# in3otd/glfer

Measured on NVIDIA B200. Metric: spectrogram_frames_per_sec, higher is better.
Workload: dtype f32

## Files before the change

glfer_b200/csrc/gram_common.cuh:

```cuda
#pragma once
#include <cuda_runtime.h>
#include <cstdio>
#include <cstdlib>
#include <cstring>
#include <cstdint>
#include <atomic>
#include <vector>
#include <algorithm>

#include "fft_core.cuh"
#include "fft_wpf.cuh"
#include "levels.cuh"
#include "avg_frame.cuh"
#include "tables.hpp"
#include "../../include/glb_shim.h"

using namespace glb;

extern std::atomic<unsigned long long> g_launches;
extern int g_big_pair;
extern int g_kernel_pref;
extern int g_last_family;
extern "C" void glb_set_error(const char *msg);

// ... 762 lines not shown
        last_pass_rt<M>(v, t, buf, p.tw, tr);
        if (MULTI) {
          if (w0) emit_bins_rt<M, true>(v, t, tr, sink_multi);
          else emit_bins_rt<M, false>(v, t, tr, sink_multi);
        } else {
          if (w0) emit_bins_rt<M, true>(v, t, tr, sink_single);
          else emit_bins_rt<M, false>(v, t, tr, sink_single);
        }
      } else {
        TwRegs tl;
        load_last_regs<M>(tl, t, p.tw, p.vtab);
        last_pass_load<M>(v, t, buf);
        last_pass_compute_rt<M>(v, t, tl);
        if (MULTI) {
          if (w0) emit_bins_rt<M, true>(v, t, tl, sink_multi);
          else emit_bins_rt<M, false>(v, t, tl, sink_multi);
        } else {
          if (w0) emit_bins_rt<M, true>(v, t, tl, sink_single);
          else emit_bins_rt<M, false>(v, t, tl, sink_single);
        }
      }
      if (!MULTI) {
        if constexpr (LEV) {
          if (active) store_levels<M>(lev_ptr, t, yv, p.lm);
        }
        if (!LEV || p.rows != nullptr) {
          if (db) {
#pragma unroll
            for (int slot = 0; slot < 17; slot++) yv[slot] = 10.f * log10f(yv[slot]);
          }
          if constexpr (AVG) {
            if (active && av_mask != 0) {
              float *hrow = hist + hslot * av_band - p.av.minbin;
#pragma unroll
              for (int slot = 0; slot < 17; slot++)
                if (av_mask & (1u << slot)) hrow[slot_bin<M>(t, slot)] = yv[slot];
            }
          }
          if (active && storing) {
            GLB_CHECK_ROW(p, row);
            GLB_CHECK_ROW(p, row + M);
            store_row<M>(row, t, yv);
          }
        }
      }
    }
    if (MULTI && active) {
      float *row = row_ptr;
      const bool db = p.rows_db != 0;
      if constexpr (LEV) store_levels<M>(lev_ptr, t, acc, p.lm);
      if (!LEV || p.rows != nullptr) {
#pragma unroll
        for (int slot = 0; slot < 17; slot++) {
          if (slot < 16 || t == 0) {
            float y = acc[slot];
            if (db) y = 10.f * log10f(y);
            row[slot_bin<M>(t, slot)] = y;
          }
        }
      }
    }
    slot_new = slot_next;
    if constexpr (AVG) hslot = (hslot + 1 == av_depth) ? 0 : hslot + 1;
  }
}



template <int M, int P> struct PairMidPasses {
  static __device__ __forceinline__ void run(float2 (&va)[kPoints], float2 (&vb)[kPoints], int t, float4 *buf, const TwRegs &tr) {
    if constexpr (P < Plan<M>::NP - 1) {
      pass_load2<M>(va, vb, t, buf);
      pass_compute_rt<M, P>(va, tr);
      pass_compute_rt<M, P>(vb, tr);
      __syncthreads();
      pass_scatter2<M, P>(va, vb, t, buf);
      __syncthreads();
      PairMidPasses<M, P + 1>::run(va, vb, t, buf, tr);
    }
  }
};

template <int M, int QS> struct PairGeo {
  static constexpr int T = M / kPoints, NB = kPoints >> QS, SLOTS = NB + 1, NW = (T + 31) / 32;
  static constexpr int HOP = (2 * T) << QS;
  static constexpr int G = Geo<M>::G, THREADS = Geo<M>::THREADS;
  static constexpr size_t BUF_BYTES = (size_t) BufSize<M>::value * sizeof(float4);
  static constexpr size_t RING_OFF = BUF_BYTES;
  static constexpr size_t RED_OFF = RING_OFF + (size_t) SLOTS * HOP * sizeof(float);
  static constexpr size_t MU_OFF = RED_OFF + (((size_t) (NB + 1) * NW * sizeof(float) + 15) / 16) * 16;
  static constexpr size_t MBAR_OFF = MU_OFF + (((size_t) SLOTS * sizeof(float) + 15) / 16) * 16;
  static constexpr size_t GROUP_BYTES = MBAR_OFF + 16;
  static constexpr size_t SMEM = (size_t) G * GROUP_BYTES;
  static constexpr int MINB_ = 65536 / (THREADS * 168);
  static constexpr int MINB = MINB_ < 1 ? 1 : MINB_;
};

template <int M, int QS>
__global__ void __launch_bounds__(Geo<M>::THREADS, (PairGeo<M, QS>::MINB)) gram_pair_kernel(const KParams p) {
  using PG = PairGeo<M, QS>;
  constexpr int T = PG::T, G = PG::G, N = 2 * M, NB = PG::NB, SLOTS = PG::SLOTS, NW = PG::NW, HOP = PG::HOP;
  constexpr int BQ = 1 << QS;
  constexpr int W = T < 32 ? T : 32;
  extern __shared__ __align__(16) unsigned char smem_raw[];
  const int g = threadIdx.x / T;
  const int t = threadIdx.x % T;
  unsigned char *gbase = smem_raw + (size_t) g * PG::GROUP_BYTES;
  float4 *buf = reinterpret_cast<float4 *>(gbase);
  float *ring = reinterpret_cast<float *>(gbase + PG::RING_OFF);
  float *red = reinterpret_cast<float *>(gbase + PG::RED_OFF);
  float *mu = reinterpret_cast<float *>(gbase + PG::MU_OFF);
  unsigned long long *mbar = reinterpret_cast<unsigned long long *>(gbase + PG::MBAR_OFF);
  const long long gid = (long long) blockIdx.x * G + g;
  const long long fb = gid * p.frames_per_group;
  const bool group_active = fb < p.nframes;
  const long long f_first = p.first_frame + fb;
  const bool sub = p.fused_mean != 0;
  constexpr unsigned blk_bytes = (unsigned) HOP * 4u;
  unsigned phase = 0;

  TwRegs tr;
  load_tw_regs<M>(tr, t, p.tw, p.vtab);

  if (t == 0) {
    mbar_init(mbar, 1);
    asm volatile("fence.mbarrier_init.release.cluster;" ::: "memory");
  }
  __syncthreads();

  {
    const long long b0 = f_first - (NB - 1);
    const bool b_there = fb + 1 < p.nframes;
    unsigned bytes = 0;
#pragma unroll
    for (int lb = 0; lb <= NB; lb++) {
      const long long blk = b0 + lb;
      const bool want = group_active && blk >= 0 && (lb < NB || b_there);
      if (!want) {
        float2 *z = reinterpret_cast<float2 *>(ring + (size_t) lb * HOP);
#pragma unroll
        for (int i = 0; i < BQ; i++) z[t + T * i] = make_float2(0.f, 0.f);
      } else {
        bytes += blk_bytes;
      }
    }
    if (bytes != 0) {
      if (t == 0) {
        mbar_expect_tx(mbar, bytes);
#pragma unroll
        for (int lb = 0; lb <= NB; lb++) {
          const long long blk = b0 + lb;
          if (blk >= 0 && (lb < NB || b_there))
            tma_load_1d(ring + (size_t) lb * HOP, p.samples + (blk * HOP - p.origin), blk_bytes, mbar);
        }
      }
      mbar_wait(mbar, phase);
      phase ^= 1;
    }
    __syncthreads();
    if (sub) {
#pragma unroll
      for (int lb = 0; lb < NB - 1; lb++) {
        const float m = ring_block_mean<M>(ring + (size_t) lb * HOP, QS, t, red + lb * NW, p.inv_hop_mean, g);
        if (t == 0) mu[lb] = m;
      }
      __syncthreads();
    }
  }

  int s0 = 0;
  bool pending = false;
  for (int it = 0; it < p.frames_per_group; it += 2) {
    const long long fl = fb + it;
    const bool active_a = fl < p.nframes, active_b = fl + 1 < p.nframes;
    const long long f = p.first_frame + fl;
    if (pending) {
      mbar_wait(mbar, phase);
      phase ^= 1;
    }
    int slot_of[NB + 1];
#pragma unroll
    for (int lb = 0; lb <= NB; lb++) slot_of[lb] = (s0 + lb) % SLOTS;

    float2 va[kPoints], vb[kPoints];
    {
      float2 x[kPoints + BQ];
#pragma unroll
      for (int lb = 0; lb <= NB; lb++) {
        const float2 *bp = reinterpret_cast<const float2 *>(ring + (size_t) slot_of[lb] * HOP);
#pragma unroll
        for (int i = 0; i < BQ; i++) x[lb * BQ + i] = bp[t + T * i];
      }
      float m[NB + 1];
#pragma unroll
      for (int lb = 0; lb <= NB; lb++) m[lb] = 0.f;
      if (sub) {
        float sn[2];
#pragma unroll
        for (int e = 0; e < 2; e++) {
          float a = 0.f;
#pragma unroll
          for (int i = 0; i < BQ; i++) {
            const float2 c = x[(NB - 1 + e) * BQ + i];
            a += c.x + c.y;
          }
#pragma unroll
          for (int o = W / 2; o > 0; o >>= 1) a += __shfl_xor_sync(0xffffffffu, a, o);
          sn[e] = a;
        }
        if (NW > 1) {
          if ((t & 31) == 0) {
            red[t >> 5] = sn[0];
            red[NW + (t >> 5)] = sn[1];
          }
          __syncthreads();
        }
        m[NB - 1] = ring_block_total<M>(sn[0], red, p.inv_hop_mean);
        m[NB] = ring_block_total<M>(sn[1], red + NW, p.inv_hop_mean);
#pragma unroll
        for (int lb = 0; lb < NB - 1; lb++) m[lb] = mu[slot_of[lb]];
        if (t == 0) {
          mu[slot_of[NB - 1]] = m[NB - 1];
          mu[slot_of[NB]] = m[NB];
        }
      }
      const float2 *w2 = reinterpret_cast<const float2 *>(p.tapers);
#pragma unroll
      for (int q = 0; q < kPoints; q++) {
        const float2 w = ld_taper(w2 + t + T * q);
        va[q] = mul2(sub2(x[q], bc(m[q >> QS])), w);
        vb[q] = mul2(sub2(x[q + BQ], bc(m[(q >> QS) + 1])), w);
      }
    }
    pass_compute_rt<M, 0>(va, tr);
    pass_compute_rt<M, 0>(vb, tr);
    __syncthreads();
    pass_scatter2<M, 0>(va, vb, t, buf);
    {
      const bool next_a = (it + 2 < p.frames_per_group) && (fl + 2 < p.nframes);
      const bool next_b = next_a && (fl + 3 < p.nframes);
      pending = next_a;
      if (next_a && t == 0) {
        asm volatile("fence.proxy.async.shared::cta;" ::: "memory");
        mbar_expect_tx(mbar, next_b ? 2 * blk_bytes : blk_bytes);
        tma_load_1d(ring + (size_t) slot_of[0] * HOP, p.samples + ((f + 2) * (long long) HOP - p.origin), blk_bytes, mbar);
        if (next_b)
          tma_load_1d(ring + (size_t) slot_of[1] * HOP, p.samples + ((f + 3) * (long long) HOP - p.origin), blk_bytes, mbar);
      }
    }
    __syncthreads();
    PairMidPasses<M, 1>::run(va, vb, t, buf, tr);
    last_pass_load2<M>(va, vb, t, buf);
    const bool db = p.rows_db != 0;
    const bool w0 = t < 32;
#pragma unroll
    for (int e = 0; e < 2; e++) {
      float2 *v = e == 0 ? va : vb;
      last_pass_compute_rt<M>(v, t, tr);
      float yv[17];
      yv[16] = 1.f;
      auto sink = [&](int slot, float2 a, bool) { yv[slot] = norm2(a); };
      if (w0) emit_bins_rt<M, true>(v, t, tr, sink);
      else emit_bins_rt<M, false>(v, t, tr, sink);
      if (db) {
#pragma unroll
        for (int slot = 0; slot < 17; slot++) yv[slot] = 10.f * log10f(yv[slot]);
      }
      if (e == 0 ? active_a : active_b) store_row<M>(p.rows + (fl + e) * p.row_stride, t, yv);
    }
    s0 = (s0 + 2) % SLOTS;
  }
}

#ifndef GLB_WPF_MINB
#define GLB_WPF_MINB 5
#endif
constexpr int kWpfWarps = 2;

template <int M, int QW>
__device__ __forceinline__ void wpf_remove_means(float2 (&x)[kWP], float inv_hop) {
  constexpr int T = Wpf<M>::T, NB = kWP >> QW;
#pragma unroll
  for (int b = 0; b < NB; b++) {
    float s = 0.f;
#pragma unroll
    for (int q = b << QW; q < (b + 1) << QW; q++) s += x[q].x + x[q].y;
#pragma unroll
    for (int o = T / 2; o > 0; o >>= 1) s += __shfl_xor_sync(0xffffffffu, s, o);
    const float m = s * inv_hop;
#pragma unroll
    for (int q = b << QW; q < (b + 1) << QW; q++) {
      x[q].x -= m;
      x[q].y -= m;
    }
  }
}

template <int M>
__global__ void __launch_bounds__(32 * kWpfWarps, GLB_WPF_MINB) gram_wpf_kernel(const KParams p) {
  constexpr int T = Wpf<M>::T, N = 2 * M, FPW = 32 / T;
  extern __shared__ __align__(16) unsigned char smem_raw[];
  const int warp = threadIdx.x >> 5, lane = threadIdx.x & 31;
  const int g = lane / T, t = lane % T;
  float2 *tile = reinterpret_cast<float2 *>(smem_raw) + (size_t) (warp * FPW + g) * (Wpf<M>::TILE + 2);
  const long long gid = ((long long) blockIdx.x * kWpfWarps + warp) * FPW + g;
  const long long fb = gid * p.frames_per_group;

  WpfRegs rg;
  wpf_load_regs<M>(rg, t, p.roots, p.vtab);
  const float2 *w2 = reinterpret_cast<const float2 *>(p.tapers) + t;
  const bool db = p.rows_db != 0;

  for (int it = 0; it < p.frames_per_group; ++it) {
    const long long fl = fb + it;
    const bool active = fl < p.nframes;
    const long long fe = active ? fl : (p.nframes - 1);
    const long long f = p.first_frame + fe;
    const float2 *src = reinterpret_cast<const float2 *>(p.samples + (f * (long long) p.hop - p.n_ov - p.origin)) + t;
    float2 v[kWP];
#pragma unroll
    for (int q = 0; q < kWP; q++) v[q] = ldg2(src + T * q);
    if (fl + 1 < p.nframes && it + 1 < p.frames_per_group) {
      const float *nx = p.samples + ((f + 1) * (long long) p.hop - p.origin);
      for (int i = t * 32; i < p.hop; i += T * 32) asm volatile("prefetch.global.L2 [%0];" ::"l"(nx + i));
    }
    if (p.fused_mean) {
      switch (p.qs) {
        case 6: wpf_remove_means<M, 6>(v, p.inv_hop_mean); break;
        case 5: wpf_remove_means<M, 5>(v, p.inv_hop_mean); break;
        case 4: wpf_remove_means<M, 4>(v, p.inv_hop_mean); break;
        case 3: wpf_remove_means<M, 3>(v, p.inv_hop_mean); break;
        default: wpf_remove_means<M, 2>(v, p.inv_hop_mean); break;
      }
    }
#pragma unroll
    for (int q = 0; q < kWP; q++) {
      const float2 w = ldg2(w2 + T * q);
      v[q].x *= w.x;
      v[q].y *= w.y;
    }
    wpf_pass_a<M>(v);
    __syncwarp();
    wpf_scatter<M>(v, t, tile);
    __syncwarp();
    wpf_gather<M>(v, t, tile);
    wpf_pass_b<M>(v, t, rg);
    float *row = p.rows + fe * p.row_stride;
    wpf_emit<M>(v, t, rg, [&](int, int bin, float2 a, bool) {
      float y = norm2(a);
      if (db) y = 10.f * log10f(y);
      if (active) row[bin] = y;
    });
  }
}

template <int M>
inline int launch_wpf(const KParams &kp, cudaStream_t st) {
  int dev = 0, sms = 0;
  CU(cudaGetDevice(&dev));
  CU(cudaDeviceGetAttribute(&sms, cudaDevAttrMultiProcessorCount, dev));
  constexpr int FPW = 32 / Wpf<M>::T;
  const size_t smem = (size_t) kWpfWarps * FPW * (Wpf<M>::TILE + 2) * sizeof(float2);
  static thread_local int occ_cache[64];
  int &occ = occ_cache[dev & 63];
  if (occ == 0) {
    CU(cudaFuncSetAttribute(gram_wpf_kernel<M>, cudaFuncAttributeMaxDynamicSharedMemorySize, 227 * 1024));
    CU(cudaOccupancyMaxActiveBlocksPerMultiprocessor(&occ, gram_wpf_kernel<M>, 32 * kWpfWarps, smem));
    if (occ < 1) occ = 1;
  }
  long long groups = (long long) sms * occ * kWpfWarps * FPW;
  if (groups > kp.nframes) groups = kp.nframes;
  if (groups < 1) groups = 1;
  KParams k = kp;
  k.frames_per_group = (int) ((kp.nframes + groups - 1) / groups);
  const long long used = (kp.nframes + k.frames_per_group - 1) / k.frames_per_group;
  const int ctas = (int) ((used + kWpfWarps * FPW - 1) / (kWpfWarps * FPW));
  gram_wpf_kernel<M><<<ctas, 32 * kWpfWarps, smem, st>>>(k);
  CU(cudaGetLastError());
  g_launches++;
  g_last_family = 3;
  return GLB_OK;
}


template <int M>
inline int launch_gram_m(const KParams &kp, bool multi, int groups_hint, cudaStream_t st, int allow) {
  using GeoM = Geo<M>;
  int dev = 0, sms = 0;
  CU(cudaGetDevice(&dev));
  CU(cudaDeviceGetAttribute(&sms, cudaDevAttrMultiProcessorCount, dev));
  const bool plain = multi || (kp.ra9mb_a <= 0.f && kp.limiter == 0);
  if constexpr (M >= 256 && M <= 2048) {
    constexpr int unitw = 2 * Wpf<M>::T;
    int qw = -1;
    for (int s2 = 2; s2 <= 6; s2++)
      if (kp.hop == (unitw << s2)) qw = s2;
    const bool mean_ok = !kp.fused_mean || (qw >= 0 && (kp.n_ov % kp.hop) == 0);
    const bool pref_ok = (allow & 4) != 0;
    if (pref_ok && !multi && plain && kp.rows != nullptr && kp.levels == nullptr && kp.spectrum == nullptr && kp.means == nullptr && mean_ok &&
        (kp.hop % 2) == 0 && ((kp.n_ov + kp.origin) % 2) == 0 && ((reinterpret_cast<uintptr_t>(kp.samples) & 7) == 0)) {
      const long long lo_s = kp.origin > 0 ? kp.origin : 0;
      long long f_lo = (lo_s + kp.n_ov + kp.hop - 1) / kp.hop;
      long long f_hi = (kp.origin + kp.count - kp.hop) / kp.hop + 1;
      if (f_lo < kp.first_frame) f_lo = kp.first_frame;
      if (f_hi > kp.first_frame + kp.nframes) f_hi = kp.first_frame + kp.nframes;
      if (f_hi > f_lo) {
        KParams kw = kp;
        kw.qs = qw;
        kw.first_frame = f_lo;
        kw.nframes = f_hi - f_lo;
        kw.rows = kp.rows + (f_lo - kp.first_frame) * kp.row_stride;
        int rc = launch_wpf<M>(kw, st);
        if (rc != GLB_OK) return rc;
        KParams ke = kp;
        if (f_lo > kp.first_frame) {
          ke.nframes = f_lo - kp.first_frame;
          rc = launch_gram_m<M>(ke, multi, groups_hint, st, 1);
          if (rc != GLB_OK) return rc;
        }
        if (f_hi < kp.first_frame + kp.nframes) {
          ke = kp;
          ke.first_frame = f_hi;
          ke.nframes = kp.first_frame + kp.nframes - f_hi;
          ke.rows = kp.rows + (f_hi - kp.first_frame) * kp.row_stride;
          rc = launch_gram_m<M>(ke, multi, groups_hint, st, 1);
          if (rc != GLB_OK) return rc;
        }
        return GLB_OK;
      }
    }
  }
  {
    const int unit = 2 * GeoM::T;
    int qs = -1;
    for (int s2 = 0; s2 <= 4; s2++)
      if (kp.hop == (unit << s2)) qs = s2;
    const long long blk_lo = (kp.first_frame - kp.n_ov / kp.hop) * (long long) kp.hop;
    const long long blk_hi = (kp.first_frame + kp.nframes) * (long long) kp.hop;
    const bool covered = kp.origin <= (blk_lo > 0 ? blk_lo : 0) && blk_hi <= kp.origin + kp.count;
    const bool regular = qs >= 0 && (kp.n_ov % kp.hop) == 0 && (kp.hop % 4) == 0 && (kp.origin % 4) == 0 &&
                         ((reinterpret_cast<uintptr_t>(kp.samples) & 15) == 0) && covered;
    if constexpr (GeoM::RT && M >= 256) {
      if (regular && !multi && plain && kp.rows != nullptr && kp.levels == nullptr && kp.spectrum == nullptr && kp.means == nullptr &&
          (allow & 8) != 0 && (qs == 3 || qs == 2) && kp.nframes >= 2) {
        void (*pk)(const KParams) = qs == 3 ? gram_pair_kernel<M, 3> : gram_pair_kernel<M, 2>;
        const size_t smem = qs == 3 ? PairGeo<M, 3>::SMEM : PairGeo<M, 2>::SMEM;
        static thread_local int occ_pair[2][64];
        int &occ = occ_pair[qs - 2][dev & 63];
        if (occ == 0) {
          CU(cudaFuncSetAttribute(pk, cudaFuncAttributeMaxDynamicSharedMemorySize, (int) smem));
          CU(cudaOccupancyMaxActiveBlocksPerMultiprocessor(&occ, pk, GeoM::THREADS, smem));
          if (occ < 1) occ = -1;
        }
        if (occ >= 1) {
          long long groups = groups_hint > 0 ? groups_hint : (long long) sms * occ * GeoM::G;
          if (groups > (kp.nframes + 1) / 2) groups = (kp.nframes + 1) / 2;
          if (groups < 1) groups = 1;
          KParams k = kp;
          k.qs = qs;
          long long fpg = (kp.nframes + groups - 1) / groups;
          fpg += fpg & 1;
          k.frames_per_group = (int) fpg;
          long long used = (kp.nframes + fpg - 1) / fpg;
          int ctas = (int) ((used + GeoM::G - 1) / GeoM::G);
          pk<<<ctas, GeoM::THREADS, smem, st>>>(k);
          CU(cudaGetLastError());
          g_launches++;
          g_last_family = 4;
          return GLB_OK;
        }
      }
    }
    if (regular && plain && (kp.rows != nullptr || kp.levels != nullptr) && kp.spectrum == nullptr && kp.means == nullptr &&
        (allow & 2) != 0) {
      const int nb = kPoints >> qs;
      const bool avg = kp.av_on != 0;
      const int hist_floats = avg ? kp.av.depth * (kp.av.maxbin - kp.av.minbin) : 0;
      const RingLayout L = ring_layout<M>(kp.hop, nb, hist_floats);
      size_t smem = (size_t) GeoM::G * L.group_bytes + ((multi ? RingGeo<M, true>::RT : RingGeo<M, false>::RT) ? 0 : Geo<M>::TWS_BYTES);
      if (const char *e = getenv("GLB_SMEM_PAD_KB")) smem += (size_t) atoi(e) * 1024;
      if (smem <= 227 * 1024) {
        void (*rk)(const KParams) = nullptr;
        const bool lev = kp.levels != nullptr;
        if (avg) {
          if constexpr (M == 2048 || M == 4096) {
            if (multi || lev) { glb_set_error("glb_launch_gram: fused averaging is for periodogram float rows"); return GLB_EINVAL; }
            rk = qs == 3 ? gram_ring_kernel<M, false, 3, false, true>
                         : (qs == 2 ? gram_ring_kernel<M, false, 2, false, true> : gram_ring_kernel<M, false, -1, false, true>);
            CU(cudaFuncSetAttribute(rk, cudaFuncAttributeMaxDynamicSharedMemorySize, 227 * 1024));
            int occ_a = 0;
            CU(cudaOccupancyMaxActiveBlocksPerMultiprocessor(&occ_a, rk, GeoM::THREADS, smem));
            if (occ_a < 1) { glb_set_error("glb_launch_gram: fused averaging does not fit shared memory"); return GLB_EINVAL; }
            long long groups = groups_hint > 0 ? groups_hint : (long long) sms * occ_a;
            if (groups > kp.nframes) groups = kp.nframes;
            if (groups < 1) groups = 1;
            KParams k = kp;
            k.qs = qs;
            k.frames_per_group = (int) ((kp.nframes + groups - 1) / groups);
            const long long used = (kp.nframes + k.frames_per_group - 1) / k.frames_per_group;
            rk<<<(int) used, GeoM::THREADS, smem, st>>>(k);
            CU(cudaGetLastError());
            g_launches++;
            g_last_family = 2;
            return GLB_OK;
          } else {
            glb_set_error("glb_launch_gram: fused averaging is available for N = 4096 and 8192 (see glb_gram_fused_avg_ok)");
            return GLB_EINVAL;
          }
        }
        if (qs == 3) rk = multi ? (lev ? gram_ring_kernel<M, true, 3, true> : gram_ring_kernel<M, true, 3, false>)
                                : (lev ? gram_ring_kernel<M, false, 3, true> : gram_ring_kernel<M, false, 3, false>);
        else if (qs == 2) rk = multi ? (lev ? gram_ring_kernel<M, true, 2, true> : gram_ring_kernel<M, true, 2, false>)
                                     : (lev ? gram_ring_kernel<M, false, 2, true> : gram_ring_kernel<M, false, 2, false>);
        else rk = multi ? (lev ? gram_ring_kernel<M, true, -1, true> : gram_ring_kernel<M, true, -1, false>)
                        : (lev ? gram_ring_kernel<M, false, -1, true> : gram_ring_kernel<M, false, -1, false>);
        static thread_local int occ_ring[2][2][5][64];
        int &occ = occ_ring[lev ? 1 : 0][multi ? 1 : 0][qs][dev & 63];
        if (occ == 0) {
          CU(cudaFuncSetAttribute(rk, cudaFuncAttributeMaxDynamicSharedMemorySize, 227 * 1024));
          CU(cudaOccupancyMaxActiveBlocksPerMultiprocessor(&occ, rk, GeoM::THREADS, smem));
          if (occ < 1) occ = -1;
        }
        int occ_generic_bound = (int) ((227 * 1024) / GeoM::smem_bytes(false));
        const bool worth = occ >= 2 || (occ >= 1 && occ_generic_bound <= 1) || GeoM::THREADS >= 512 || g_kernel_pref == 2;
        if (occ >= 1 && worth) {
          long long groups = groups_hint > 0 ? groups_hint : (long long) sms * occ * GeoM::G;
          constexpr int kRingWaves = 4, kRingMinRun = 16;
          if (groups_hint <= 0 && occ >= 2) {
            int waves = kRingWaves;
            while (waves > 1 && kp.nframes < groups * waves * kRingMinRun) waves--;
            groups *= waves;
          }
          if (groups > kp.nframes) groups = kp.nframes;
          if (groups < 1) groups = 1;
          KParams k = kp;
          k.qs = qs;
          k.frames_per_group = (int) ((kp.nframes + groups - 1) / groups);
          long long used = (kp.nframes + k.frames_per_group - 1) / k.frames_per_group;
          int ctas = (int) ((used + GeoM::G - 1) / GeoM::G);
          rk<<<ctas, GeoM::THREADS, smem, st>>>(k);
          CU(cudaGetLastError());
          g_launches++;
          g_last_family = 2;
          return GLB_OK;
        }
      }
    }
  }
  if (kp.av_on) {
    glb_set_error("glb_launch_gram: fused averaging needs the regular geometry of the ring kernel (see glb_gram_fused_avg_ok)");
    return GLB_EINVAL;
  }
  const int variant = multi ? 2 : (plain ? 1 : 0);
  const bool glev = kp.levels != nullptr;
  if (glev && !plain) {
    glb_set_error("glb_launch_gram: display levels are not available together with RA9MB / limiter");
    return GLB_EINVAL;
  }
  auto kern = glev ? (multi ? gram_kernel<M, true, true, true> : gram_kernel<M, false, true, true>)
                   : (multi ? gram_kernel<M, true, true> : (plain ? gram_kernel<M, false, true> : gram_kernel<M, false, false>));
  const size_t smem = GeoM::smem_bytes(multi);
  static thread_local int occ_cache[6][64];
  int &occ = occ_cache[variant + (glev ? 3 : 0)][dev & 63];
  if (occ == 0) {
    CU(cudaFuncSetAttribute(kern, cudaFuncAttributeMaxDynamicSharedMemorySize, 227 * 1024));
    CU(cudaOccupancyMaxActiveBlocksPerMultiprocessor(&occ, kern, GeoM::THREADS, smem));
    if (occ < 1) occ = 1;
  }
  long long groups = groups_hint > 0 ? groups_hint : (long long) sms * occ * GeoM::G;
  if (groups > kp.nframes) groups = kp.nframes;
  if (groups < 1) groups = 1;
  KParams k = kp;
  k.frames_per_group = (int) ((kp.nframes + groups - 1) / groups);
  long long used = (kp.nframes + k.frames_per_group - 1) / k.frames_per_group;
  int ctas = (int) ((used + GeoM::G - 1) / GeoM::G);
  k.fused_mean = 0;
  k.qs = 0;
  if (kp.fused_mean) {
    const int unit = 2 * GeoM::T;
    int qs = -1;
    for (int s2 = 0; s2 <= 4; s2++)
      if (kp.hop == (unit << s2)) qs = s2;
    if (qs >= 0 && (k.n_ov % kp.hop) == 0) {
      k.fused_mean = 1;
      k.qs = qs;
    } else {
      glb_set_error("glb_launch_gram: fused block means need hop = (N/16) << s, s = 0..4");
      return GLB_EINVAL;
    }
  }
  kern<<<ctas, GeoM::THREADS, smem, st>>>(k);
  CU(cudaGetLastError());
  g_launches++;
  g_last_family = 1;
  return GLB_OK;
}


#define GLB_DECLARE_PART(K) int glb_gram_part_##K(int m, const KParams &k, bool multi, int groups_hint, cudaStream_t st, int allow)
GLB_DECLARE_PART(0);
GLB_DECLARE_PART(1);
GLB_DECLARE_PART(2);
GLB_DECLARE_PART(3);
int glb_gram_big(int m, const KParams &k, bool multi, int groups_hint, cudaStream_t st, bool small_too);
```

glfer_b200/csrc/gram_kernels.cu:

```cuda
#include "gram_common.cuh"

static thread_local char g_err[512] = "";
std::atomic<unsigned long long> g_launches{0};
int g_kernel_pref = 0;
int g_last_family = 0;
int g_force_generic = 0;

extern "C" const char *glb_last_error(void) { return g_err; }
extern "C" void glb_set_error(const char *msg) { snprintf(g_err, sizeof g_err, "%s", msg ? msg : ""); }
extern "C" unsigned long long glb_kernel_launches(void) { return g_launches.load(); }
extern "C" void glb_force_generic_kernel(int on) { g_force_generic = on; }
extern "C" void glb_set_kernel_preference(int pref) {
  g_big_pair = pref != 6;
  g_kernel_pref = pref == 6 ? 0 : pref;
}
extern "C" int glb_last_kernel_family(void) { return g_last_family; }

extern "C" int glb_device_count(int *count) {
  int c = 0;
  cudaError_t e = cudaGetDeviceCount(&c);
  if (e != cudaSuccess) {
    snprintf(g_err, sizeof g_err, "cudaGetDeviceCount: %s", cudaGetErrorString(e));
    *count = 0;
    return GLB_ENODEV;
// ... 162 lines not shown
    return GLB_EINVAL;
  }
  if (a->nframes <= 0) return GLB_OK;
  const GramTables *tb = (const GramTables *) a->tables;
  if (tb->n != a->n) {
    glb_set_error("glb_launch_gram: tables were built for another FFT size");
    return GLB_EINVAL;
  }
  KParams k;
  memset(&k, 0, sizeof k);
  k.samples = a->samples;
  k.origin = a->origin;
  k.count = a->count;
  k.tapers = a->tapers;
  k.ntapers = a->ntapers;
  k.taper_sym = a->ntapers == 1 && a->taper_symmetric;
  k.means = a->block_means;
  k.means_first_block = a->means_first_block;
  k.fused_mean = a->fused_mean;
  k.hop = a->hop;
  k.n_ov = a->n - a->hop;
  k.cblk = (k.n_ov + a->hop - 1) / a->hop;
  k.inv_hop = (float) (1.0 / (double) a->hop);
  k.inv_hop_mean = (float) (1.0 / (double) a->hop);
  k.ra9mb_a = a->ra9mb_a;
  k.limiter = a->limiter;
  k.zero_hist = a->zero_history;
  k.lim_scale = (float) pow((double) a->taper_scale, 0.9);
  k.spec_scale = (float) (1.0 / (2.0 * (double) a->taper_scale));
  k.first_frame = a->first_frame;
  k.nframes = a->nframes;
  k.rows = a->rows;
  k.row_stride = a->row_stride;
  k.rows_db = a->rows_db;
  k.spectrum = (float2 *) a->spectrum;
  k.tw = tb->tw;
  k.vtab = tb->vtab;
  k.roots = tb->roots;
  if (a->levels) {
    if (!a->level_tables) {
      glb_set_error("glb_launch_gram: levels output needs level_tables");
      return GLB_EINVAL;
    }
    if (a->spectrum) {
      glb_set_error("glb_launch_gram: levels and spectrum outputs are exclusive");
      return GLB_EINVAL;
    }
    k.levels = a->levels;
    k.lev_stride = a->levels_stride;
    k.lm.thr = ((const LevelTables *) a->level_tables)->thr_f;
    k.lm.lut = a->levels_log ? a->level_lut : nullptr;
    k.lm.log_scale = a->levels_log;
    k.lm.dmin = a->level_min;
    k.lm.dmax = a->level_max;
    k.lm.thr_level = a->level_thr;
  }
  if (a->fused_avg) {
    const glb_avg_args *av = (const glb_avg_args *) a->fused_avg;
    if (!av->band_only || av->out_double || av->first_frame != a->first_frame || av->nframes != a->nframes || !av->avg_rows ||
        !glb_gram_fused_avg_ok(a->n, a->hop, av->depth, av->maxbin - av->minbin) || a->origin % 4 != 0) {
      glb_set_error("glb_launch_gram: fused averaging not available for this launch");
      return GLB_EINVAL;
    }
    k.av_on = 1;
    k.av = *av;
  }
  if (!a->rows && !a->levels && !a->spectrum) {
    glb_set_error("glb_launch_gram: no output requested");
    return GLB_EINVAL;
  }
  const bool multi = a->ntapers > 1;
  if (multi && a->spectrum) {
    glb_set_error("glb_launch_gram: spectrum output is only defined for one taper");
    return GLB_EINVAL;
  }
  if (a->fused_mean && a->block_means) {
    glb_set_error("glb_launch_gram: fused_mean and block_means are exclusive");
    return GLB_EINVAL;
  }
  cudaStream_t st = (cudaStream_t) stream;
  int allow = 3;
  if (g_force_generic || g_kernel_pref == 1 || a->zero_history || a->general_only) allow = 1;
  else if (g_kernel_pref == 3) allow = 7;
  else if (g_kernel_pref == 4) allow = 11;
  const int m = a->n / 2;
  int rc = -1;
  if ((g_kernel_pref == 0 || g_kernel_pref == 5) && !g_force_generic && !a->general_only) rc = glb_gram_big(m, k, multi, a->groups_hint, st, g_kernel_pref == 5);
  if (rc != -1) return rc;
  rc = glb_gram_part_0(m, k, multi, a->groups_hint, st, allow);
  if (rc == -1) rc = glb_gram_part_1(m, k, multi, a->groups_hint, st, allow);
  if (rc == -1) rc = glb_gram_part_2(m, k, multi, a->groups_hint, st, allow);
  if (rc == -1) rc = glb_gram_part_3(m, k, multi, a->groups_hint, st, allow);
  if (rc != -1) return rc;
  return GLB_EINVAL;
}

__global__ void block_means_kernel(const float *__restrict__ samples, long long origin, long long count,
                                   int hop, long long first_block, long long nblocks, float *__restrict__ means) {
  const int lane = threadIdx.x & 31;
  const long long warp = ((long long) blockIdx.x * blockDim.x + threadIdx.x) >> 5;
  const long long nwarps = ((long long) gridDim.x * blockDim.x) >> 5;
  for (long long b = warp; b < nblocks; b += nwarps) {
    const long long base = (first_block + b) * hop - origin;
    float s = 0.f;
    for (int i = lane; i < hop; i += 32) {
      const long long r = base + i;
      s += (r >= 0 && r < count) ? __ldg(samples + r) : 0.f;
    }
#pragma unroll
    for (int o = 16; o > 0; o >>= 1) s += __shfl_xor_sync(0xffffffffu, s, o);
    if (lane == 0) means[b] = s / (float) hop;
  }
}

extern "C" int glb_launch_block_means(const float *samples, long long origin, long long count, int hop,
                                      long long first_block, long long nblocks, float *means, void *stream) {
  if (nblocks <= 0) return GLB_OK;
  if (hop < 1) { glb_set_error("block_means: hop < 1"); return GLB_EINVAL; }
  const int threads = 256;
  long long ctas = (nblocks * 32 + threads - 1) / threads;
  if (ctas > 148 * 16) ctas = 148 * 16;
  block_means_kernel<<<(int) ctas, threads, 0, (cudaStream_t) stream>>>(samples, origin, count, hop, first_block, nblocks, means);
  CU(cudaGetLastError());
  g_launches++;
  return GLB_OK;
}

__global__ void pcm16_to_float_kernel(const short *__restrict__ in, float *__restrict__ out, long long n) {
  const long long stride = (long long) gridDim.x * blockDim.x;
  for (long long i = (long long) blockIdx.x * blockDim.x + threadIdx.x; i < n; i += stride)
    out[i] = (float) in[i] / 32768.f;
}
__global__ void pcm8_to_float_kernel(const unsigned char *__restrict__ in, float *__restrict__ out, long long n) {
  const long long stride = (long long) gridDim.x * blockDim.x;
  for (long long i = (long long) blockIdx.x * blockDim.x + threadIdx.x; i < n; i += stride)
    out[i] = ((float) in[i] - 128.f) / 128.f;
}
extern "C" int glb_launch_pcm16_to_float(const short *pcm, float *out, long long count, void *stream) {
  if (count <= 0) return GLB_OK;
  long long ctas = std::min<long long>((count + 255) / 256, 148 * 32);
  pcm16_to_float_kernel<<<(int) ctas, 256, 0, (cudaStream_t) stream>>>(pcm, out, count);
  CU(cudaGetLastError());
  g_launches++;
  return GLB_OK;
}
extern "C" int glb_launch_pcm8_to_float(const unsigned char *pcm, float *out, long long count, void *stream) {
  if (count <= 0) return GLB_OK;
  long long ctas = std::min<long long>((count + 255) / 256, 148 * 32);
  pcm8_to_float_kernel<<<(int) ctas, 256, 0, (cudaStream_t) stream>>>(pcm, out, count);
  CU(cudaGetLastError());
  g_launches++;
  return GLB_OK;
}

struct AvgRed {
  double mx; int arg; double sum; double mn;
};

template <typename OutT>
__global__ void __launch_bounds__(256) avg_kernel(const glb_avg_args a, int chunk) {
  extern __shared__ double cum[];
  __shared__ double s_mx[8], s_sum[8], s_mn[8], s_var[8];
  __shared__ int s_arg[8], s_cnt[8];
  __shared__ double b_mx, b_sum, b_mn, b_var;
  __shared__ int b_arg, b_cnt;
  const int tid = threadIdx.x, lane = tid & 31, wid = tid >> 5;
  const int band = a.maxbin - a.minbin;
// ... 816 lines not shown
```

glfer_b200/csrc/iq.cu:

```cuda
#include "gram_common.cuh"
#include "iq_core.cuh"

extern int g_force_generic;
int glb_tables_get(const void *tables, int *n, const float2 **tw, const float2 **vtab);

constexpr float kIqPowerScale = 8.f;

template <int M, int QSC, bool LEV = false>
__global__ void __launch_bounds__(Geo<M>::THREADS, (RingGeo<M, false>::MINB)) gram_iq_kernel(const KParams p) {
  using GeoM = Geo<M>;
  constexpr int T = GeoM::T, G = GeoM::G;
  constexpr bool RT = RingGeo<M, false>::RT;
  extern __shared__ __align__(16) unsigned char smem_raw[];
  const int g = threadIdx.x / T;
  const int t = threadIdx.x % T;
  const int qs = QSC >= 0 ? QSC : p.qs;
  const int hop = QSC >= 0 ? ((2 * T) << (QSC >= 0 ? QSC : 0)) : p.hop;
  const int nb = kPoints >> qs;
  const RingLayout L = ring_layout<M>(hop, nb);
  const int slots = L.slots;
  unsigned char *gbase = smem_raw + (size_t) g * L.group_bytes;
  float2 *buf = reinterpret_cast<float2 *>(gbase);
  float *ring = reinterpret_cast<float *>(gbase + L.ring_off);
  float *red = reinterpret_cast<float *>(gbase + L.red_off);
// ... 88 lines not shown
      pass_compute_rt<M, 0>(v, tr);
      group_sync<M>(g);
      pass_scatter<M, 0>(v, t, buf);
    } else {
      group_sync<M>(g);
      pass_store<M, 0>(v, t, buf, p.tw);
    }
    if (!GLB_RING_EXTRA && next_there && t == 0) request_next();
    group_sync<M>(g);
    RingMidPasses<M, 1, RT>::run(v, t, buf, tw_mid, tr, g);
    float yv[17];
    yv[16] = 0.f;
    const bool w0 = t < 32;
    if constexpr (RT) {
      last_pass_rt<M>(v, t, buf, p.tw, tr);
    } else {
      TwRegs tl;
      load_last_regs<M>(tl, t, p.tw, p.vtab);
      last_pass_load<M>(v, t, buf);
      last_pass_compute_rt<M>(v, t, tl);
    }
    if (w0) iq_emit_power<M, true>(v, t, kIqPowerScale, yv);
    else iq_emit_power<M, false>(v, t, kIqPowerScale, yv);
    if constexpr (LEV) {
      if (active) {
#pragma unroll
        for (int slot = 0; slot < 17; slot++) {
          if (slot == 16) {
            if (t == 0) lev_ptr[M - 1] = map_level(yv[16], p.lm);
          } else if (slot != 1 || t != 0) {
            lev_ptr[iq_pixel_offset<M>(ob, slot)] = map_level(yv[slot], p.lm);
          }
        }
      }
      lev_ptr += p.lev_stride;
    } else if (active) {
      GLB_CHECK_ROW(p, row_ptr);
      GLB_CHECK_ROW(p, row_ptr + M - 1);
#pragma unroll
      for (int slot = 0; slot < 17; slot++) {
        if (slot == 16) {
          if (t == 0) st_row(row_ptr, yv[16]);
        } else if (slot != 1 || t != 0) {
          st_row(row_ptr + iq_slot_offset<M>(ob, slot), yv[slot]);
        }
      }
    }
    slot_new = slot_next;
  }
}

template <int M>
static int launch_iq_fused(const KParams &kp, cudaStream_t st) {
  using GeoM = Geo<M>;
  constexpr bool RT = RingGeo<M, false>::RT;
  const int unit = 2 * GeoM::T;
  int qs = -1;
  for (int s2 = 0; s2 <= 4; s2++)
    if (kp.hop == (unit << s2)) qs = s2;
  if (qs < 0 || (kp.n_ov % kp.hop) != 0 || (kp.hop % 4) != 0 || (kp.origin % 4) != 0 ||
      (reinterpret_cast<uintptr_t>(kp.samples) & 15) != 0)
    return 0;
  const long long blk_lo = (kp.first_frame - kp.n_ov / kp.hop) * (long long) kp.hop;
  const long long blk_hi = (kp.first_frame + kp.nframes) * (long long) kp.hop;
  if (!(kp.origin <= (blk_lo > 0 ? blk_lo : 0) && blk_hi <= kp.origin + kp.count)) return 0;
  const RingLayout L = ring_layout<M>(kp.hop, kPoints >> qs);
  const size_t smem = (size_t) GeoM::G * L.group_bytes + (RT ? 0 : Geo<M>::TWS_BYTES);
  if (smem > 227 * 1024) return 0;
  const bool lev = kp.levels != nullptr;
  void (*rk)(const KParams) = lev ? (qs == 3 ? gram_iq_kernel<M, 3, true> : (qs == 2 ? gram_iq_kernel<M, 2, true> : gram_iq_kernel<M, -1, true>))
                                  : (qs == 3 ? gram_iq_kernel<M, 3> : (qs == 2 ? gram_iq_kernel<M, 2> : gram_iq_kernel<M, -1>));
  int dev = 0, sms = 0;
  CU(cudaGetDevice(&dev));
  CU(cudaDeviceGetAttribute(&sms, cudaDevAttrMultiProcessorCount, dev));
  static thread_local int occ_iq[2][5][64];
  int &occ = occ_iq[lev][qs][dev & 63];
  if (occ == 0) {
    CU(cudaFuncSetAttribute(rk, cudaFuncAttributeMaxDynamicSharedMemorySize, 227 * 1024));
    CU(cudaOccupancyMaxActiveBlocksPerMultiprocessor(&occ, rk, GeoM::THREADS, smem));
    if (occ < 1) occ = -1;
  }
  if (occ < 1) return 0;
  long long groups = (long long) sms * occ * GeoM::G;
  constexpr int kRingWaves = 4, kRingMinRun = 16;
  if (occ >= 2) {
    int waves = kRingWaves;
    while (waves > 1 && kp.nframes < groups * waves * kRingMinRun) waves--;
    groups *= waves;
  }
  if (groups > kp.nframes) groups = kp.nframes;
  if (groups < 1) groups = 1;
  KParams k = kp;
  k.qs = qs;
  k.frames_per_group = (int) ((kp.nframes + groups - 1) / groups);
  const long long used = (kp.nframes + k.frames_per_group - 1) / k.frames_per_group;
  const int ctas = (int) ((used + GeoM::G - 1) / GeoM::G);
  rk<<<ctas, GeoM::THREADS, smem, st>>>(k);
  CU(cudaGetLastError());
  g_launches++;
  g_last_family = 2;
  return 1;
}

static int iq_fused_n(int n) { return n >= 32 && n <= 8192 && (n & (n - 1)) == 0; }

static bool iq_fused_geometry(int n, int hop) {
  if (!iq_fused_n(n) || hop < 1 || hop > n || (n - hop) % hop != 0) return false;
  for (int s = 0; s <= 4; s++)
    if (hop == ((n / 16) << s)) return true;
  return false;
}

static bool iq_fused_allowed() { return g_force_generic == 0 && g_kernel_pref != 1; }

extern "C" long long glb_iq_gram_scratch_bytes(int n, int hop, long long nframes, int levels) {
  if (nframes <= 0 || (iq_fused_allowed() && iq_fused_geometry(n, hop))) return 0;
  return nframes * ((long long) (n + 1) * 2 + (levels ? n : 0)) * (long long) sizeof(float);
}

extern "C" int glb_launch_iq_gram(const glb_iq_gram_args *a, void *stream) {
  if (!a || !a->tables || !a->samples || !a->taper || !a->rows == !a->levels || a->n < 32 || a->n > 16384 ||
      (a->n & (a->n - 1)) != 0 || a->hop < 1 || a->hop > a->n || a->origin < 0 || a->count < 0 || a->first_frame < 0) {
    glb_set_error("glb_launch_iq_gram: invalid arguments (exactly one of rows and levels)");
    return GLB_EINVAL;
  }
  if (a->levels && (!a->level_tables || a->levels_stride != a->n)) {
    glb_set_error("glb_launch_iq_gram: levels need level_tables and levels_stride = n");
    return GLB_EINVAL;
  }
  if (a->nframes <= 0) return GLB_OK;
  int tn = 0;
  const float2 *tw = nullptr, *vtab = nullptr;
  if (glb_tables_get(a->tables, &tn, &tw, &vtab) != GLB_OK || tn != 2 * a->n) {
    glb_set_error("glb_launch_iq_gram: tables must be built for 2 n");
    return GLB_EINVAL;
  }
  if (iq_fused_allowed() && iq_fused_geometry(a->n, a->hop)) {
    KParams k;
    memset(&k, 0, sizeof k);
    k.samples = a->samples;
    k.origin = 2 * a->origin;
    k.count = 2 * a->count;
    k.tapers = a->taper;
    k.ntapers = 1;
    k.hop = 2 * a->hop;
    k.n_ov = 2 * (a->n - a->hop);
    k.first_frame = a->first_frame;
    k.nframes = a->nframes;
    k.rows = a->rows;
    k.row_stride = a->n;
    if (a->levels) {
      k.levels = a->levels;
      k.lev_stride = a->levels_stride;
      k.lm.thr = ((const LevelTables *) a->level_tables)->thr_f;
      k.lm.lut = a->levels_log ? a->level_lut : nullptr;
      k.lm.log_scale = a->levels_log;
      k.lm.dmin = a->level_min;
      k.lm.dmax = a->level_max;
      k.lm.thr_level = a->level_thr;
    }
    k.tw = tw;
    k.vtab = vtab;
    cudaStream_t st = (cudaStream_t) stream;
    int rc = 0;
    switch (a->n) {
      case 32: rc = launch_iq_fused<32>(k, st); break;
      case 64: rc = launch_iq_fused<64>(k, st); break;
// ... 26 lines not shown
```

Before: 210.3 million.

## Replace TMA shared-memory ring in pair kernel with direct global loads and L2 prefetch

The pair FFT kernel no longer stages sample blocks through a TMA-fed shared-memory ring with mbarriers. It loads each block directly from global memory with ldg and issues a bulk L2 prefetch for the next two blocks. Block means are now held in registers (mc) instead of shared memory. Freeing that shared memory allows a fixed minimum of 4 blocks per SM. The pair kernel is also enabled by default for M=2048, qs=3 when there are enough frames, and the grid is scaled by multiple waves. This trades shared-memory staging for redundant global/L2 reads of overlapping blocks in exchange for higher occupancy and less synchronisation.

```diff
diff --git a/glfer_b200/csrc/gram_common.cuh b/glfer_b200/csrc/gram_common.cuh
--- a/glfer_b200/csrc/gram_common.cuh
+++ b/glfer_b200/csrc/gram_common.cuh
@@ -868,24 +868,20 @@
 };
 
 template <int M, int QS> struct PairGeo {
-  static constexpr int T = M / kPoints, NB = kPoints >> QS, SLOTS = NB + 1, NW = (T + 31) / 32;
+  static constexpr int T = M / kPoints, NB = kPoints >> QS, NW = (T + 31) / 32;
   static constexpr int HOP = (2 * T) << QS;
   static constexpr int G = Geo<M>::G, THREADS = Geo<M>::THREADS;
   static constexpr size_t BUF_BYTES = (size_t) BufSize<M>::value * sizeof(float4);
-  static constexpr size_t RING_OFF = BUF_BYTES;
-  static constexpr size_t RED_OFF = RING_OFF + (size_t) SLOTS * HOP * sizeof(float);
-  static constexpr size_t MU_OFF = RED_OFF + (((size_t) (NB + 1) * NW * sizeof(float) + 15) / 16) * 16;
-  static constexpr size_t MBAR_OFF = MU_OFF + (((size_t) SLOTS * sizeof(float) + 15) / 16) * 16;
-  static constexpr size_t GROUP_BYTES = MBAR_OFF + 16;
+  static constexpr size_t RED_OFF = BUF_BYTES;
+  static constexpr size_t GROUP_BYTES = RED_OFF + (((size_t) (NB + 1) * NW * sizeof(float) + 15) / 16) * 16;
   static constexpr size_t SMEM = (size_t) G * GROUP_BYTES;
-  static constexpr int MINB_ = 65536 / (THREADS * 168);
-  static constexpr int MINB = MINB_ < 1 ? 1 : MINB_;
+  static constexpr int MINB = 4;
 };
 
 template <int M, int QS>
 __global__ void __launch_bounds__(Geo<M>::THREADS, (PairGeo<M, QS>::MINB)) gram_pair_kernel(const KParams p) {
   using PG = PairGeo<M, QS>;
-  constexpr int T = PG::T, G = PG::G, N = 2 * M, NB = PG::NB, SLOTS = PG::SLOTS, NW = PG::NW, HOP = PG::HOP;
+  constexpr int T = PG::T, NB = PG::NB, NW = PG::NW, HOP = PG::HOP;
   constexpr int BQ = 1 << QS;
   constexpr int W = T < 32 ? T : 32;
   extern __shared__ __align__(16) unsigned char smem_raw[];
@@ -893,122 +889,70 @@
   const int t = threadIdx.x % T;
   unsigned char *gbase = smem_raw + (size_t) g * PG::GROUP_BYTES;
   float4 *buf = reinterpret_cast<float4 *>(gbase);
-  float *ring = reinterpret_cast<float *>(gbase + PG::RING_OFF);
   float *red = reinterpret_cast<float *>(gbase + PG::RED_OFF);
-  float *mu = reinterpret_cast<float *>(gbase + PG::MU_OFF);
-  unsigned long long *mbar = reinterpret_cast<unsigned long long *>(gbase + PG::MBAR_OFF);
-  const long long gid = (long long) blockIdx.x * G + g;
-  const long long fb = gid * p.frames_per_group;
-  const bool group_active = fb < p.nframes;
-  const long long f_first = p.first_frame + fb;
+  const long long fb = ((long long) blockIdx.x * PG::G + g) * p.frames_per_group;
+  const long long b_end = p.first_frame + p.nframes;
   const bool sub = p.fused_mean != 0;
-  constexpr unsigned blk_bytes = (unsigned) HOP * 4u;
-  unsigned phase = 0;
 
   TwRegs tr;
   load_tw_regs<M>(tr, t, p.tw, p.vtab);
 
-  if (t == 0) {
-    mbar_init(mbar, 1);
-    asm volatile("fence.mbarrier_init.release.cluster;" ::: "memory");
-  }
-  __syncthreads();
-
-  {
-    const long long b0 = f_first - (NB - 1);
-    const bool b_there = fb + 1 < p.nframes;
-    unsigned bytes = 0;
-#pragma unroll
-    for (int lb = 0; lb <= NB; lb++) {
-      const long long blk = b0 + lb;
-      const bool want = group_active && blk >= 0 && (lb < NB || b_there);
-      if (!want) {
-        float2 *z = reinterpret_cast<float2 *>(ring + (size_t) lb * HOP);
-#pragma unroll
-        for (int i = 0; i < BQ; i++) z[t + T * i] = make_float2(0.f, 0.f);
-      } else {
-        bytes += blk_bytes;
-      }
-    }
-    if (bytes != 0) {
-      if (t == 0) {
-        mbar_expect_tx(mbar, bytes);
-#pragma unroll
-        for (int lb = 0; lb <= NB; lb++) {
-          const long long blk = b0 + lb;
-          if (blk >= 0 && (lb < NB || b_there))
-            tma_load_1d(ring + (size_t) lb * HOP, p.samples + (blk * HOP - p.origin), blk_bytes, mbar);
-        }
-      }
-      mbar_wait(mbar, phase);
-      phase ^= 1;
-    }
-    __syncthreads();
-    if (sub) {
-#pragma unroll
-      for (int lb = 0; lb < NB - 1; lb++) {
-        const float m = ring_block_mean<M>(ring + (size_t) lb * HOP, QS, t, red + lb * NW, p.inv_hop_mean, g);
-        if (t == 0) mu[lb] = m;
-      }
-      __syncthreads();
-    }
-  }
-
-  int s0 = 0;
-  bool pending = false;
+  float mc[NB - 1];
   for (int it = 0; it < p.frames_per_group; it += 2) {
     const long long fl = fb + it;
     const bool active_a = fl < p.nframes, active_b = fl + 1 < p.nframes;
     const long long f = p.first_frame + fl;
-    if (pending) {
-      mbar_wait(mbar, phase);
-      phase ^= 1;
-    }
-    int slot_of[NB + 1];
-#pragma unroll
-    for (int lb = 0; lb <= NB; lb++) slot_of[lb] = (s0 + lb) % SLOTS;
+    const long long b0 = f - (NB - 1);
+    if (t == 0 && it + 2 < p.frames_per_group && f + 2 < b_end) {
+      const unsigned bytes = (f + 3 < b_end ? 2u : 1u) * HOP * 4u;
+      asm volatile("cp.async.bulk.prefetch.L2.global [%0], %1;" ::"l"(p.samples + ((f + 2) * HOP - p.origin)), "r"(bytes) : "memory");
+    }
 
     float2 va[kPoints], vb[kPoints];
     {
       float2 x[kPoints + BQ];
 #pragma unroll
       for (int lb = 0; lb <= NB; lb++) {
-        const float2 *bp = reinterpret_cast<const float2 *>(ring + (size_t) slot_of[lb] * HOP);
-#pragma unroll
-        for (int i = 0; i < BQ; i++) x[lb * BQ + i] = bp[t + T * i];
+        const long long blk = b0 + lb;
+        if (blk >= 0 && blk < b_end) {
+          const float2 *bp = reinterpret_cast<const float2 *>(p.samples + (blk * HOP - p.origin)) + t;
+#pragma unroll
+          for (int i = 0; i < BQ; i++) x[lb * BQ + i] = ldg2(bp + T * i);
+        } else {
+#pragma unroll
+          for (int i = 0; i < BQ; i++) x[lb * BQ + i] = make_float2(0.f, 0.f);
+        }
       }
       float m[NB + 1];
 #pragma unroll
       for (int lb = 0; lb <= NB; lb++) m[lb] = 0.f;
       if (sub) {
-        float sn[2];
-#pragma unroll
-        for (int e = 0; e < 2; e++) {
-          float a = 0.f;
-#pragma unroll
-          for (int i = 0; i < BQ; i++) {
-            const float2 c = x[(NB - 1 + e) * BQ + i];
-            a += c.x + c.y;
+        const bool first = it == 0;
+        float sn[NB + 1];
+#pragma unroll
+        for (int lb = 0; lb <= NB; lb++) {
+          if (lb >= NB - 1 || first) {
+            float a = 0.f;
+#pragma unroll
+            for (int i = 0; i < BQ; i++) {
+              const float2 c = x[lb * BQ + i];
+              a += c.x + c.y;
+            }
+#pragma unroll
+            for (int o = W / 2; o > 0; o >>= 1) a += __shfl_xor_sync(0xffffffffu, a, o);
+            sn[lb] = a;
+            if (NW > 1 && (t & 31) == 0) red[lb * NW + (t >> 5)] = a;
           }
-#pragma unroll
-          for (int o = W / 2; o > 0; o >>= 1) a += __shfl_xor_sync(0xffffffffu, a, o);
-          sn[e] = a;
-        }
-        if (NW > 1) {
-          if ((t & 31) == 0) {
-            red[t >> 5] = sn[0];
-            red[NW + (t >> 5)] = sn[1];
-          }
-          __syncthreads();
-        }
-        m[NB - 1] = ring_block_total<M>(sn[0], red, p.inv_hop_mean);
-        m[NB] = ring_block_total<M>(sn[1], red + NW, p.inv_hop_mean);
-#pragma unroll
-        for (int lb = 0; lb < NB - 1; lb++) m[lb] = mu[slot_of[lb]];
-        if (t == 0) {
-          mu[slot_of[NB - 1]] = m[NB - 1];
-          mu[slot_of[NB]] = m[NB];
-        }
+        }
+        if (NW > 1) __syncthreads();
+#pragma unroll
+        for (int lb = 0; lb <= NB; lb++) {
+          if (lb >= NB - 1) m[lb] = ring_block_total<M>(sn[lb], red + lb * NW, p.inv_hop_mean);
+          else if (first) m[lb] = (b0 + lb < 0) ? 0.f : ring_block_total<M>(sn[lb], red + lb * NW, p.inv_hop_mean);
+          else m[lb] = mc[lb];
+        }
+#pragma unroll
+        for (int lb = 0; lb < NB - 1; lb++) mc[lb] = m[lb + 2];
       }
       const float2 *w2 = reinterpret_cast<const float2 *>(p.tapers);
 #pragma unroll
@@ -1022,18 +966,6 @@
     pass_compute_rt<M, 0>(vb, tr);
     __syncthreads();
     pass_scatter2<M, 0>(va, vb, t, buf);
-    {
-      const bool next_a = (it + 2 < p.frames_per_group) && (fl + 2 < p.nframes);
-      const bool next_b = next_a && (fl + 3 < p.nframes);
-      pending = next_a;
-      if (next_a && t == 0) {
-        asm volatile("fence.proxy.async.shared::cta;" ::: "memory");
-        mbar_expect_tx(mbar, next_b ? 2 * blk_bytes : blk_bytes);
-        tma_load_1d(ring + (size_t) slot_of[0] * HOP, p.samples + ((f + 2) * (long long) HOP - p.origin), blk_bytes, mbar);
-        if (next_b)
-          tma_load_1d(ring + (size_t) slot_of[1] * HOP, p.samples + ((f + 3) * (long long) HOP - p.origin), blk_bytes, mbar);
-      }
-    }
     __syncthreads();
     PairMidPasses<M, 1>::run(va, vb, t, buf, tr);
     last_pass_load2<M>(va, vb, t, buf);
@@ -1054,7 +986,6 @@
       }
       if (e == 0 ? active_a : active_b) store_row<M>(p.rows + (fl + e) * p.row_stride, t, yv);
     }
-    s0 = (s0 + 2) % SLOTS;
   }
 }
 
@@ -1168,6 +1099,7 @@
   return GLB_OK;
 }
 
+constexpr int kRingWaves = 4, kRingMinRun = 16;
 
 template <int M>
 inline int launch_gram_m(const KParams &kp, bool multi, int groups_hint, cudaStream_t st, int allow) {
@@ -1227,8 +1159,9 @@
     const bool regular = qs >= 0 && (kp.n_ov % kp.hop) == 0 && (kp.hop % 4) == 0 && (kp.origin % 4) == 0 &&
                          ((reinterpret_cast<uintptr_t>(kp.samples) & 15) == 0) && covered;
     if constexpr (GeoM::RT && M >= 256) {
+      const bool pair_auto = M == 2048 && qs == 3 && !kp.rows_db;
       if (regular && !multi && plain && kp.rows != nullptr && kp.levels == nullptr && kp.spectrum == nullptr && kp.means == nullptr &&
-          (allow & 8) != 0 && (qs == 3 || qs == 2) && kp.nframes >= 2) {
+          !kp.av_on && (allow & 8) != 0 && (g_kernel_pref == 4 || pair_auto) && (qs == 3 || qs == 2) && kp.nframes >= 2) {
         void (*pk)(const KParams) = qs == 3 ? gram_pair_kernel<M, 3> : gram_pair_kernel<M, 2>;
         const size_t smem = qs == 3 ? PairGeo<M, 3>::SMEM : PairGeo<M, 2>::SMEM;
         static thread_local int occ_pair[2][64];
@@ -1238,8 +1171,14 @@
           CU(cudaOccupancyMaxActiveBlocksPerMultiprocessor(&occ, pk, GeoM::THREADS, smem));
           if (occ < 1) occ = -1;
         }
-        if (occ >= 1) {
+        const bool fill = g_kernel_pref == 4 || kp.nframes >= 2LL * sms * (occ > 0 ? occ : 0) * GeoM::G;
+        if (occ >= 1 && fill) {
           long long groups = groups_hint > 0 ? groups_hint : (long long) sms * occ * GeoM::G;
+          if (groups_hint <= 0 && occ >= 2) {
+            int waves = kRingWaves;
+            while (waves > 1 && kp.nframes < groups * waves * kRingMinRun) waves--;
+            groups *= waves;
+          }
           if (groups > (kp.nframes + 1) / 2) groups = (kp.nframes + 1) / 2;
           if (groups < 1) groups = 1;
           KParams k = kp;
@@ -1311,7 +1250,6 @@
         const bool worth = occ >= 2 || (occ >= 1 && occ_generic_bound <= 1) || GeoM::THREADS >= 512 || g_kernel_pref == 2;
         if (occ >= 1 && worth) {
           long long groups = groups_hint > 0 ? groups_hint : (long long) sms * occ * GeoM::G;
-          constexpr int kRingWaves = 4, kRingMinRun = 16;
           if (groups_hint <= 0 && occ >= 2) {
             int waves = kRingWaves;
             while (waves > 1 && kp.nframes < groups * waves * kRingMinRun) waves--;
diff --git a/glfer_b200/csrc/gram_kernels.cu b/glfer_b200/csrc/gram_kernels.cu
--- a/glfer_b200/csrc/gram_kernels.cu
+++ b/glfer_b200/csrc/gram_kernels.cu
@@ -268,7 +268,7 @@
   int allow = 3;
   if (g_force_generic || g_kernel_pref == 1 || a->zero_history || a->general_only) allow = 1;
   else if (g_kernel_pref == 3) allow = 7;
-  else if (g_kernel_pref == 4) allow = 11;
+  else if (g_kernel_pref == 4 || g_kernel_pref == 0) allow = 11;
   const int m = a->n / 2;
   int rc = -1;
   if ((g_kernel_pref == 0 || g_kernel_pref == 5) && !g_force_generic && !a->general_only) rc = glb_gram_big(m, k, multi, a->groups_hint, st, g_kernel_pref == 5);
diff --git a/glfer_b200/csrc/iq.cu b/glfer_b200/csrc/iq.cu
--- a/glfer_b200/csrc/iq.cu
+++ b/glfer_b200/csrc/iq.cu
@@ -194,7 +194,6 @@
   }
   if (occ < 1) return 0;
   long long groups = (long long) sms * occ * GeoM::G;
-  constexpr int kRingWaves = 4, kRingMinRun = 16;
   if (occ >= 2) {
     int waves = kRingWaves;
     while (waves > 1 && kp.nframes < groups * waves * kRingMinRun) waves--;
```

Result: slower. 207.2 million, median of 6 (-1.5%).
